# passcod/zarc

Hardware: AMD Instinct MI355X
Metric: uncompressed GiB/s (pack) at zstd -3 (higher is better)
Workload: dtype u8; 1 GPU; zarc pack 10000 x 1048576 B synthetic entries per GPU, zstd level 3, checksum on (BASELINE configs[1]); entries_per_gpu=10000, entries_total=10000, entry_bytes=1048576, level=3, kinds=text/records/lz/random round-robin

## Files before the change

zarc_amd/csrc/zge_match.hip:

```cpp
#include "zarc_device.h"
#include "zarc_kernels.h"

namespace {

#ifdef ZARC_HIPEMU
#define ZGE_CLOCK() 0ull
#else
#define ZGE_CLOCK() ((unsigned long long)__builtin_readcyclecounter())
#endif
#define ZGE_IDX(u) ((uint32_t)((wave * PER + (u)) * 64 + lane))
#ifndef ZGE_S2_DUPMASK
#define ZGE_S2_DUPMASK 0
#endif
#define ZGE_PROF(i) do { if ((dbg & 1024) && tid == 0) { const unsigned long long now_ = ZGE_CLOCK(); L.prof[i] += now_ - tprev; tprev = now_; } } while (0)

constexpr int TILE = 1024;
constexpr int THREADS = 512;
constexpr int WAVES = THREADS / 64;
constexpr int PER = TILE / THREADS;
static_assert(PER == 2, "the kernel is written for two positions per thread");
constexpr int CHUNKS = TILE / 64;
constexpr int TAG_BITS = 10;
constexpr uint32_t TAG_MASK = (1u << TAG_BITS) - 1;
struct U128 { uint64_t lo, hi; };
constexpr int CAP_MAX = 256;
constexpr int REP_BACK_MAX = 256;
constexpr int TB_BYTES = 12 + REP_BACK_MAX + TILE + CAP_MAX + 24;

template <int TAB_LOG, bool NEAR16> struct MatchLds {
    static constexpr int TAB_WORDS = NEAR16 ? (1 << TAB_LOG) / 2 : 2 << TAB_LOG;
    uint32_t tab[TAB_WORDS + (NEAR16 ? 1 : 0)];
    uint32_t a0[TILE], a1[TILE];
    uint32_t ex[TILE];
    uint32_t tb[2][(TB_BYTES + 3) / 4];
    uint32_t wcnt[CHUNKS];
    uint32_t wrep[2 * CHUNKS];
    uint32_t ctrl[16];
    unsigned long long prof[15];
};
enum { K_POS = 0, K_REP0 = 1, K_REP1 = 2, K_FLAG = 3, K_SLOT = 4, K_ANY = 5, K_CHG = 6 ,
       K_CEND = 10 ,
       K_CLEN = 11 ,
       K_LONG = 12 , K_LONG2 = 13  };

__device__ __forceinline__ uint32_t hash_long32(uint64_t v)
{
    const uint32_t lo = (uint32_t)v, hi = (uint32_t)(v >> 32);
    return lo * 0x9E3779B1u + hi * 0x85EBCA77u;
}
__device__ __forceinline__ uint32_t hash_far32(uint64_t v, uint32_t w) { return hash_long32(v) + w * 0xC2B2AE3Du; }
__device__ __forceinline__ uint32_t hash_short32(uint64_t v, int nbytes)
{
    uint32_t lo = (uint32_t)v, hi = (uint32_t)(v >> 32);
    if (nbytes < 8) hi &= (nbytes > 4) ? ((1u << (8 * (nbytes - 4))) - 1) : 0u;
    if (nbytes < 4) lo &= (1u << (8 * nbytes)) - 1;
    return lo * 0xC2B2AE3Du + hi * 0x27D4EB2Fu;
}

constexpr int REP_COST = 9;
constexpr int F_REP_BACK = 256, F_BACK_CAP = 8, F_LAZY_DELTA = 5, F_MIN_REP = 3, F_SEG_LOG = 21;
template <int MATCH_COST, int LITC> __device__ __forceinline__ int32_t score_mc(uint32_t len, uint32_t off, bool is_rep)
{
    static_assert(LITC == 5 || LITC == 6, "literal cost");
    const int32_t lits = (int32_t)((len << 2) + (LITC == 6 ? len << 1 : len));
    return is_rep ? lits - REP_COST : lits - MATCH_COST - zd::hb32(off);
}
#define score_of(P_, len_, off_, rep_) score_mc<MATCH_COST, LITC>((len_), (off_), (rep_))

template <bool WIDE> __device__ __forceinline__ uint32_t match_pack_w(uint32_t off, uint32_t len, bool rep) { return off | (len << 21) | ((rep ? 1u : 0u) << (WIDE ? 31 : 30)); }
__device__ __forceinline__ uint32_t match_off(uint32_t m) { return m & 0x1FFFFFu; }
template <bool WIDE> __device__ __forceinline__ uint32_t match_len_w(uint32_t m) { return (m >> 21) & (WIDE ? 0x3FFu : 0x1FFu); }
template <bool WIDE> __device__ __forceinline__ bool match_rep_w(uint32_t m) { return WIDE ? (m >> 31) != 0 : ((m >> 30) & 1u) != 0; }
#define match_pack(o_, l_, r_) match_pack_w<(CONT_CAP > 0 || EXT_ROUND)>((o_), (l_), (r_))
#define match_len(m_) match_len_w<(CONT_CAP > 0 || EXT_ROUND)>(m_)
#define match_rep(m_) match_rep_w<(CONT_CAP > 0 || EXT_ROUND)>(m_)
constexpr int LONG_CAP = 960;

__device__ __forceinline__ uint32_t wave_match_ext(const uint8_t *src, uint32_t p, uint32_t off, uint32_t from, uint32_t maxlen, int lane)
{
    static_assert(LONG_CAP <= 1024, "one trip of 64 x 16 bytes");
    const uint32_t at = from + 16u * (uint32_t)lane;
    const bool act = at < maxlen;
    U128 a{0, 0}, b{0, 0};
    if (act) { __builtin_memcpy(&a, src + (p + at), 16); __builtin_memcpy(&b, src + (p - off + at), 16); }
    const uint64_t xl = a.lo ^ b.lo, xh = a.hi ^ b.hi;
    const uint32_t mis = xl ? (uint32_t)(zd::ctz64(xl) >> 3) : (xh ? 8u + (uint32_t)(zd::ctz64(xh) >> 3) : 16u);
    const uint64_t bad = zd::ballot(act && mis < 16u);
    uint32_t len = maxlen;
    if (bad) {
        const uint32_t first = (uint32_t)zd::ctz64(bad);
        len = from + 16u * first + zd::readlane(mis, first);
        if (len > maxlen) len = maxlen;
    }
    return len;
}

struct StageWin { const uint32_t *w; int ndw; uint32_t wofs; };
static_assert((TB_BYTES + 3) / 4 <= THREADS, "one staged dword per thread");
__device__ __forceinline__ StageWin stage_window(const ZgeParams &P, const uint8_t *src, uint32_t n, uint32_t tile, uint32_t tend, uint32_t cap_max)
{
    (void)P;
    const uint32_t before = (uint32_t)F_REP_BACK + 8;
    const uint32_t lo = tile >= before ? tile - before : 0;
    uint32_t hi = tend + cap_max + 16;
    if (hi > n + 16) hi = n + 16;
    const uintptr_t a = (uintptr_t)(src + lo);
    const uint32_t mis = (uint32_t)(a & 3);
    StageWin s;
    s.w = (const uint32_t *)(a - mis);
    s.ndw = (int)((hi - lo + mis + 3) / 4);
    s.wofs = mis - lo;
    return s;
}

__device__ __forceinline__ uint32_t tile_end(uint32_t tile, uint32_t n)
{
    uint32_t e = tile + TILE;
    const uint32_t be = (tile / ZARC_BLOCK + 1) * ZARC_BLOCK;
    if (e > be) e = be;
    return e > n ? n : e;
}

}

template <int TAB_LOG, int SHORT_BYTES, int MATCH_COST, int F_FAR_LOG, int FAR_WAYS, bool FAR_SHORT, int FAR_STEP_LOG, int FAR_RES_LOG, int FAR_SKIP, int FAR_BACK, bool DIAG,
          bool NEAR16, int FAR_CDC, int LITC, int LAZY2, bool REP_PASS, int CONT_CAP, bool EXT_ROUND>
__device__ __forceinline__ void zge_match_body(MatchLds<TAB_LOG, NEAR16> &L, const ZgeParams &P, const uint8_t *__restrict__ src_base, const uint64_t *__restrict__ src_off,
                                               const uint64_t *__restrict__ src_len, const uint32_t *__restrict__ order, const uint32_t *__restrict__ units, uint32_t n_units,
                                               const uint64_t *__restrict__ block_prefix, ZgeBlock *__restrict__ blocks,
                                               uint64_t *__restrict__ seq_scratch, uint8_t *__restrict__ lit_scratch, uint32_t *__restrict__ queue,
                                               uint32_t *__restrict__ far_scratch)
{
    constexpr int NFAR = FAR_WAYS * (FAR_SHORT ? 2 : 1);
    constexpr int NTAB = 1 + NFAR;
    constexpr int far_shift = 32 - (F_FAR_LOG + TAG_BITS);
    constexpr uint32_t far_words = (uint32_t)(((size_t)FAR_WAYS << F_FAR_LOG) * (FAR_SHORT ? 2 : 1));
    uint32_t *const far_l = far_scratch + (size_t)blockIdx.x * far_words;
    uint32_t *const far_s = far_l + ((size_t)FAR_WAYS << F_FAR_LOG);
    constexpr uint32_t far_smask = (1u << FAR_STEP_LOG) - 1, far_rmask = (1u << FAR_RES_LOG) - 1;
    static_assert(FAR_BACK % 8 == 0 && FAR_BACK >= 8 && FAR_BACK <= 48, "backward extension of far candidates");
    static_assert(!FAR_CDC || (FAR_WAYS == 1 && !FAR_SHORT && far_shift >= FAR_CDC), "content-defined sampling: one way on the 12-byte hash");
    constexpr uint32_t cdc_mask = (1u << FAR_CDC) - 1;
    uint32_t *const Ltl = L.tab, *const Lts = L.tab + (NEAR16 ? 0 : (1 << TAB_LOG));
    typedef uint16_t __attribute__((may_alias)) u16a;
    u16a *const Lt16 = (u16a *)L.tab;
    const int tid = (int)threadIdx.x, lane = zd::lane_id();
    const uint32_t dbg = DIAG ? (uint32_t)P.dbg : 0u;
    const int wave = (int)zd::uniform((uint32_t)zd::wave_id());
    const uint64_t lt = (1ull << lane) - 1;
    const uint32_t seg_mask = (1u << F_SEG_LOG) - 1;
    const uint32_t cap_max = (uint32_t)(P.cap < CAP_MAX ? P.cap : CAP_MAX);
    unsigned long long tprev = ZGE_CLOCK();
    if (tid < 15) L.prof[tid] = 0;

    constexpr uint32_t SEG_BLOCKS = (1u << F_SEG_LOG) / ZARC_BLOCK;
    for (;;) {
    if (tid == 0) L.ctrl[K_SLOT] = atomicAdd(queue, 1u);
    zd::lds_barrier();
    const uint32_t unit = L.ctrl[K_SLOT];
    if (unit >= n_units) break;
    const uint32_t slot = units[2 * unit], ub0 = units[2 * unit + 1];
    const uint32_t f = order[slot];
    const uint8_t *src = src_base + src_off[f];
    const uint32_t n = (uint32_t)src_len[f];
    const uint32_t window = n <= (1u << P.window_log) ? (n ? n : 1u) : (1u << P.window_log);
    const uint32_t hash_end = n >= 8 ? n - 7 : 0;
    const bool far_on = NFAR && n > (uint32_t)P.far_min_frame;
    const uint32_t far_end = (far_on && n >= 12) ? n - 11 : 0;
    const uint64_t first_block = block_prefix[slot];
    const uint32_t nblocks = (uint32_t)(block_prefix[slot + 1] - first_block);

    for (int i = tid; i < MatchLds<TAB_LOG, NEAR16>::TAB_WORDS; i += THREADS) L.tab[i] = 0;
    if (NFAR && far_on) {
        uint4 *f4 = (uint4 *)far_l;
        for (uint32_t i = (uint32_t)tid; i < far_words / 4; i += THREADS) f4[i] = make_uint4(0, 0, 0, 0);
        zd::wait_vmem();
    }
    if (tid == 0) { L.ctrl[K_REP0] = 0; L.ctrl[K_REP1] = 0; }
    zd::lds_barrier();
    uint32_t cold = 0, skip_left = 0;
    constexpr bool FAR_COMPACT = FAR_RES_LOG > 0 && !FAR_CDC;
    constexpr int FNEXT_ROWS = FAR_COMPACT ? 1 : PER;
    uint32_t fnext[FNEXT_ROWS][NFAR ? NFAR : 1];
    uint32_t pf_far_tile = 0xFFFFFFFFu;
    uint32_t hfn[PER] = {0xFFFFFFFFu, 0xFFFFFFFFu};
    uint32_t pf_word = 0, pf_tile = 0xFFFFFFFFu;
    uint32_t lds_tile[2] = {0xFFFFFFFFu, 0xFFFFFFFFu};
#pragma unroll
    for (int u = 0; u < FNEXT_ROWS; u++)
#pragma unroll
        for (int k = 0; k < (NFAR ? NFAR : 1); k++) fnext[u][k] = 0;

    const uint32_t ub1 = (n > ZARC_SPLIT_MIN && ub0 + SEG_BLOCKS < nblocks) ? ub0 + SEG_BLOCKS : nblocks;
    for (uint32_t b = ub0; b < ub1; b++) {
        const uint32_t bs = b * ZARC_BLOCK;
        const uint32_t be = n - bs > ZARC_BLOCK ? bs + ZARC_BLOCK : n;
        const uint32_t blen = (uint32_t)(be - bs);
        ZgeBlock *rec = blocks + first_block + b;
        uint64_t *seq_out = seq_scratch + (first_block + b) * zge_seq_stride((uint32_t)P.slot_bytes);
        uint8_t *lit_out = lit_scratch + (first_block + b) * zge_lit_stride((uint32_t)P.slot_bytes);

        if (b > ub0 && (bs & seg_mask) == 0) {
            for (int i = tid; i < MatchLds<TAB_LOG, NEAR16>::TAB_WORDS; i += THREADS) L.tab[i] = 0;
            if (NFAR) {
                uint4 *f4 = (uint4 *)far_l;
                for (uint32_t i = (uint32_t)tid; i < far_words / 4; i += THREADS) f4[i] = make_uint4(0, 0, 0, 0);
                zd::wait_vmem();
                pf_far_tile = 0xFFFFFFFFu;
            }
        }
        if (tid == 0) { L.ctrl[K_FLAG] = 0; L.ctrl[K_POS] = 0; if (CONT_CAP) L.ctrl[K_CEND] = 0xFFFFFFFFu; }
        zd::lds_barrier();
        const uint8_t first = blen ? src[bs] : 0;
        const uint64_t pat = 0x0101010101010101ull * first;
        const uint64_t *w = (const uint64_t *)(src + bs);
        if (blen >= 1024 && tid < 128 && w[tid] != pat) L.ctrl[K_FLAG] = 1;
        zd::lds_barrier();
        if (L.ctrl[K_FLAG] == 0) {
            bool diff = false;
            const uint32_t nw = blen / 8;
            for (uint32_t i = (uint32_t)tid; i < nw; i += THREADS) diff |= w[i] != pat;
            for (uint32_t i = nw * 8 + (uint32_t)tid; i < blen; i += THREADS) diff |= src[bs + i] != first;
            if (diff) L.ctrl[K_FLAG] = 1;
        }
        zd::lds_barrier();
        const bool all_same = L.ctrl[K_FLAG] == 0;
        if (tid == 0) {
            rec->frame = f; rec->index = b; rec->src_len = blen; rec->nseq = 0; rec->nlit = 0;
            rec->type = (all_same && blen >= 2) ? 1u : 2u; rec->out_len = 0; rec->pad = 0;
        }
        if (all_same && blen >= 2) { zd::lds_barrier(); continue; }

        uint32_t nseq = 0, lp = 0;

        for (uint32_t tile = bs; tile < be; tile += TILE) {
            const uint32_t tend = be - tile > TILE ? tile + TILE : be;
            const uint32_t tcount = (uint32_t)(tend - tile);
            const uint32_t segbase = tile & ~seg_mask;
            zd::lds_barrier();
            ZGE_PROF(0);
            const uint32_t pos = bs + L.ctrl[K_POS];
            const bool cont = CONT_CAP && L.ctrl[K_CEND] == L.ctrl[K_POS] && pos >= tile;
            if (pos >= tend) { if (NFAR) zd::wait_vmem(); continue; }
            if (skip_left) {
                skip_left--;
                const uint32_t start = (uint32_t)((pos > tile ? pos : tile) - tile);
                {
                    const uint32_t cntb = tcount - start, k = (uint32_t)tid * 16;
                    const uint8_t *sp = src + tile + start;
                    uint8_t *dp = lit_out + lp;
                    if (!(dbg & 32)) {
                        if (k + 16 <= cntb) { U128 v; __builtin_memcpy(&v, sp + k, 16); __builtin_memcpy(dp + k, &v, 16); }
                        else for (uint32_t r = k; r < cntb; r++) dp[r] = sp[r];
                    }
                }
                lp += tcount - start;
                if (NFAR) zd::wait_vmem();
                zd::lds_barrier();
                if (tid == 0) L.ctrl[K_POS] = (uint32_t)(tend - bs);
                continue;
            }
            const uint32_t erep0 = L.ctrl[K_REP0], erep1 = L.ctrl[K_REP1];
            if (CONT_CAP && cont) {
                const uint32_t idx_c = pos - tile;
                if (wave == (int)(idx_c >> 7)) {
                    const uint32_t limit = (uint32_t)(be - pos);
                    uint32_t clen = 0;
                    if (erep0 != 0 && erep0 <= pos && erep0 <= window) clen = wave_match_ext(src, pos, erep0, 0, limit < (uint32_t)CONT_CAP ? limit : (uint32_t)CONT_CAP, lane);
                    if (lane == 0) L.ctrl[K_CLEN] = clen;
                }
            }
            if (tid == 0) L.ctrl[K_ANY] = 0;
            if (REP_PASS && tid < 4) L.ctrl[K_CHG + tid] = 0;
            if (EXT_ROUND && tid == 0) { L.ctrl[K_LONG] = 0; L.ctrl[K_LONG2] = 0; }

            const uint32_t bsel = (tile / TILE) & 1u;
            const uint8_t *const tbb = (const uint8_t *)L.tb[bsel];
            const uint8_t *const tbn = (const uint8_t *)L.tb[bsel ^ 1u];
            const StageWin sw = stage_window(P, src, n, tile, tend, cap_max);
            const uint32_t wofs = sw.wofs;
            const uint32_t ntile = tile + TILE;
            uint32_t wofs_n = 0;
            bool staged_now = false;
            {
                if (lds_tile[bsel] != tile) {
                    uint32_t v = pf_word;
                    if (pf_tile != tile && tid < sw.ndw) v = sw.w[tid];
                    if (tid < sw.ndw) L.tb[bsel][tid] = v;
                    lds_tile[bsel] = tile;
                    staged_now = true;
                }
                if (ntile < n) {
                    const StageWin nw = stage_window(P, src, n, ntile, tile_end(ntile, n), cap_max);
                    wofs_n = nw.wofs;
                    uint32_t v = pf_word;
                    if (pf_tile != ntile && tid < nw.ndw) v = nw.w[tid];
                    if (tid < nw.ndw) L.tb[bsel ^ 1u][tid] = v;
                    lds_tile[bsel ^ 1u] = ntile;
                    const uint32_t n2 = ntile + TILE;
                    if (n2 < n) {
                        const StageWin w2 = stage_window(P, src, n, n2, tile_end(n2, n), cap_max);
                        if (tid < w2.ndw) pf_word = w2.w[tid];
                        pf_tile = n2;
                    }
// ... 4 lines not shown
            uint64_t p8[PER];
            uint32_t fe[PER][NFAR ? NFAR : 1], ftag[PER][FAR_SHORT ? 2 : 1];
            uint32_t foffs[PER][NFAR ? NFAR : 1];
            uint64_t qf[PER][NFAR ? NFAR : 1];
            const bool far_ahead = NFAR && pf_far_tile == tile;
#pragma unroll
            for (int u = 0; u < PER; u++) {
                const uint32_t idx = ZGE_IDX(u);
                const uint32_t p = tile + idx;
                uint32_t hl = 0xFFFFFFFFu, hs = 0xFFFFFFFFu;
                p8[u] = 0;
#pragma unroll
                for (int k = 0; k < (NFAR ? NFAR : 1); k++) {
                    if (FAR_COMPACT) {
                        const uint32_t got = zd::shfl(fnext[0][k], (int)(((uint32_t)u * 64u + (uint32_t)lane) >> FAR_RES_LOG));
                        fe[u][k] = (far_ahead && !(idx & far_rmask)) ? got : 0u;
                    } else fe[u][k] = far_ahead ? fnext[FAR_COMPACT ? 0 : u][k] : 0u;
                    foffs[u][k] = 0; qf[u][k] = 0;
                }
                ftag[u][0] = 0xFFFFFFFFu;
                if (FAR_SHORT) ftag[u][1] = 0xFFFFFFFFu;
                uint32_t hfc = 0xFFFFFFFFu;
                if (idx < tcount) {
                    p8[u] = zd::load_u64(tbb + (uint32_t)(p + wofs));
                    if (p < hash_end && !(dbg & 64)) {
                        const uint32_t h32s = hash_short32(p8[u], SHORT_BYTES);
                        const uint32_t h32l = NEAR16 ? 0u : hash_long32(p8[u]);
                        hl = NEAR16 ? 0xFFFFFFFFu : h32l >> (32 - (TAB_LOG + TAG_BITS));
                        hs = NEAR16 ? h32s >> (32 - TAB_LOG) : h32s >> (32 - (TAB_LOG + TAG_BITS));
                        if (FAR_CDC) {
                            if (p < far_end && !(dbg & 2048)) {
                                if (far_ahead) hfc = hfn[u];
                                else {
                                    const uint32_t w8 = zd::load_u32(tbb + (uint32_t)(p + 8 + wofs));
                                    const uint32_t h32f = hash_far32(p8[u], w8);
                                    if (((h32f >> (far_shift - FAR_CDC)) & cdc_mask) == 0 && !((uint32_t)p8[u] == (uint32_t)(p8[u] >> 32) && (uint32_t)p8[u] == w8)) hfc = h32f >> far_shift;
                                }
                            }
                            if (hfc != 0xFFFFFFFFu) {
                                if (!far_ahead) fe[u][0] = zd::load_l2_u32(far_l + (size_t)(hfc >> TAG_BITS));
                                else {
                                    const uint32_t e = fe[u][0];
                                    uint32_t o = (e && (e & TAG_MASK) == (hfc & TAG_MASK) && !(dbg & 4096)) ? p - (segbase + (e >> TAG_BITS) - 1) : 0u;
                                    if (o + 8 > p || o > window || (dbg & 1)) o = 0;
                                    foffs[u][0] = o;
                                    if (o) qf[u][0] = zd::load_u64(src + (p - o));
                                }
                            }
                        } else
                        if (NFAR && p < far_end && !(p & far_rmask) && !(dbg & 2048)) {
                            const uint32_t hf = (h32l + zd::load_u32(tbb + (uint32_t)(p + 8 + wofs)) * 0xC2B2AE3Du) >> far_shift, hg = h32s >> far_shift;
                            ftag[u][0] = hf & TAG_MASK;
                            if (FAR_SHORT) ftag[u][1] = hg & TAG_MASK;
                            if (!far_ahead) {
                                if (FAR_WAYS == 2) {
                                    const uint64_t el = zd::load_l2_u64(far_l + (size_t)(hf >> TAG_BITS) * 2);
                                    fe[u][0] = (uint32_t)el; fe[u][1] = (uint32_t)(el >> 32);
                                    if (FAR_SHORT) { const uint64_t es = zd::load_l2_u64(far_s + (size_t)(hg >> TAG_BITS) * 2); fe[u][2] = (uint32_t)es; fe[u][3] = (uint32_t)(es >> 32); }
                                } else {
#pragma unroll
                                for (int w = 0; w < FAR_WAYS; w++) {
                                    fe[u][w] = zd::load_l2_u32(far_l + ((size_t)(hf >> TAG_BITS) * FAR_WAYS + w));
                                    if (FAR_SHORT) fe[u][FAR_WAYS + w] = zd::load_l2_u32(far_s + ((size_t)(hg >> TAG_BITS) * FAR_WAYS + w));
                                }
                                }
                            } else {
#pragma unroll
                                for (int k = 0; k < NFAR; k++) {
                                    const uint32_t e = fe[u][k];
                                    uint32_t o = (e && (e & TAG_MASK) == ftag[u][k / (FAR_WAYS ? FAR_WAYS : 1)] && !(dbg & 4096)) ? p - (segbase + (e >> TAG_BITS) - 1) : 0u;
#pragma unroll
                                    for (int j = 0; j < k; j++) if (o == foffs[u][j]) o = 0;
                                    if (o + 8 > p || o > window || (dbg & 1)) o = 0;
                                    foffs[u][k] = o;
                                    if (o) qf[u][k] = zd::load_u64(src + (p - o));
                                }
                            }
                        }
                    }
                }
                L.a0[idx] = NEAR16 ? (hs == 0xFFFFFFFFu ? (1u << TAB_LOG) : hs) : hl;
                if (!NEAR16) L.a1[idx] = hs;
                else if (FAR_CDC) L.a1[idx] = hfc;
                L.ex[idx] = 0;
            }
            zd::lds_barrier();
            ZGE_PROF(2);
            if (NEAR16) {
              if (wave == 0 && !(dbg & 4)) {
                zd::wave_priority<3>();
                uint32_t h[CHUNKS], e[CHUNKS];
#if ZGE_S2_DUPMASK
                uint64_t dupmask = 0;
#endif
#pragma unroll
                for (int k = 0; k < CHUNKS; k++) {
                    h[k] = L.a0[k * 64 + lane];
#if ZGE_S2_DUPMASK
                    const uint32_t hn = lane < 63 ? L.a0[k * 64 + lane + 1] : 0xFFFFFFFFu;
                    if (hn == h[k]) dupmask |= 1ull << k;
#endif
                }
#pragma unroll
                for (int k = 0; k < CHUNKS; k++) {
                    e[k] = (uint32_t)Lt16[h[k]];
                    zd::wave_lds_order();
#if ZGE_S2_DUPMASK
                    if (!((dupmask >> k) & 1))
#endif
                    Lt16[h[k]] = (uint16_t)((uint32_t)tile + (uint32_t)(k * 64 + lane));
                    zd::wave_lds_order();
                }
#pragma unroll
                for (int k = 0; k < CHUNKS; k++) L.a0[k * 64 + lane] = e[k];
                zd::wave_priority<0>();
              }
            } else
            if (wave < 2 && !(dbg & 4)) {
                zd::wave_priority<3>();
                uint32_t *tab = wave == 0 ? Ltl : Lts;
                uint32_t *hc = wave == 0 ? L.a0 : L.a1;
                uint32_t h[CHUNKS], e[CHUNKS];
                uint64_t dupmask = 0;
#pragma unroll
                for (int k = 0; k < CHUNKS; k++) {
                    h[k] = hc[k * 64 + lane];
                    const uint32_t hn = lane < 63 ? hc[k * 64 + lane + 1] : 0xFFFFFFFFu;
                    if (hn == h[k]) dupmask |= 1ull << k;
                }
#pragma unroll
                for (int k = 0; k < CHUNKS; k++) {
                    const bool act = h[k] != 0xFFFFFFFFu;
                    e[k] = act ? tab[h[k] >> TAG_BITS] : 0u;
                    zd::wave_lds_order();
                    if (act && !((dupmask >> k) & 1)) {
                        const uint32_t code = ((uint32_t)(tile - segbase) + (uint32_t)(k * 64 + lane) + 1) << TAG_BITS;
                        atomicMax(&tab[h[k] >> TAG_BITS], code | (h[k] & TAG_MASK));
                    }
                    zd::wave_lds_order();
                }
#pragma unroll
                for (int k = 0; k < CHUNKS; k++)
                    hc[k * 64 + lane] = e[k] ^ (h[k] & TAG_MASK);
                zd::wave_priority<0>();
            }
            if (NFAR) zd::wait_vmem();
            zd::lds_barrier();
            ZGE_PROF(3);
            uint32_t near_e[PER] = {0, 0};
            if (FAR_CDC) {
                uint64_t vnx[PER];
                uint32_t wnx[PER];
#pragma unroll
                for (int u = 0; u < PER; u++) {
                    const uint32_t pn = ntile + ZGE_IDX(u);
                    const uint32_t at = pn < far_end ? (uint32_t)(pn + wofs_n) : 0u;
                    vnx[u] = zd::load_u64(tbn + at);
                    wnx[u] = zd::load_u32(tbn + at + 8);
                    if (NEAR16) near_e[u] = L.a0[ZGE_IDX(u)];
                }
#pragma unroll
                for (int u = 0; u < PER; u++) {
                    const uint32_t pn = ntile + ZGE_IDX(u);
                    hfn[u] = 0xFFFFFFFFu;
                    fnext[u][0] = 0;
                    if (pn < far_end && !(dbg & (2048 | 32768))) {
                        const uint64_t vn = vnx[u];
// ... 202 lines not shown
                        else { if (sc > b_score[0]) { b_score[0] = sc; b_len[0] = clen; b_off[0] = erep0; b_flags[0] = 1u | 4u; } }
                    }
                }
            }
#pragma unroll
            for (int u = 0; u < PER; u++) {
                const uint32_t idx = ZGE_IDX(u);
                const uint32_t p = tile + idx;
                const uint32_t best_len = b_len[u], best_off = b_off[u];
                const int32_t best_score = b_score[u];
                const bool best_rep = b_flags[u] & 1u, from_guess = b_flags[u] & 2u, best_fol = b_flags[u] & 4u, best_far = b_flags[u] & 8u;
                if (best_len && best_score > 0) {
                    const uint32_t q = p - best_off;
                    const uint32_t bcap = (NFAR && best_far) ? (uint32_t)FAR_BACK : (uint32_t)F_BACK_CAP;
                    uint32_t maxb = bcap;
                    if (p - bs < maxb) maxb = (uint32_t)(p - bs);
                    uint32_t back = 0;
                    if (maxb && q >= bcap && !best_fol) {
                        uint64_t best_before = q16[u].lo;
                        if (from_guess) best_before = zd::load_u64(tbb + (uint32_t)(q - 8 + wofs));
                        if (NFAR && best_far) best_before = zd::load_u64(src + (q - 8));
                        const uint64_t x = zd::load_u64(tbb + (uint32_t)(p - 8 + wofs)) ^ best_before;
                        back = x ? (uint32_t)(__clzll((long long)x) >> 3) : 8u;
                        if (NFAR && FAR_BACK > 8 && best_far) {
#pragma unroll
                            for (uint32_t j = 16; j <= (uint32_t)FAR_BACK; j += 8) {
                                if (back == j - 8 && maxb > j - 8) {
                                    const uint64_t x2 = zd::load_u64(tbb + (uint32_t)(p - j + wofs)) ^ zd::load_u64(src + (q - j));
                                    back += x2 ? (uint32_t)(__clzll((long long)x2) >> 3) : 8u;
                                }
                            }
                        }
                        if (back > maxb) back = maxb;
                    }
                    mo[u] = best_off;
                    mw[u] = best_len | (back << 16) | ((best_rep ? 1u : 0u) << 24);
                }
            }
            ZGE_PROF(11);
#pragma unroll
            for (int u = 0; u < PER; u++) L.a0[ZGE_IDX(u)] = match_pack(mo[u], mw[u] & 0xFFFF, (mw[u] >> 24) & 1);
            if (mo[0] | mo[1]) L.ctrl[K_ANY] = 1;
            if (EXT_ROUND) {
                const uint32_t r0 = (mw[0] & 0xFFFFu) + ((mw[0] >> 16) & 0xFFu), r1 = (mw[1] & 0xFFFFu) + ((mw[1] >> 16) & 0xFFu);
                if ((r0 > r1 ? r0 : r1) >= cap_max) L.ctrl[K_LONG] = 1;
            }
            uint32_t fo[PER], fw[PER];
            uint64_t msel[PER], mlit[PER];
            {
#define ZGE_FIRST 1
#include "zge_parse_round.h"
#undef ZGE_FIRST
            }
            if (EXT_ROUND && L.ctrl[K_LONG]) {
                uint64_t extm[PER];
                bool any = false;
#pragma unroll
                for (int u = 0; u < PER; u++) {
                    const uint32_t idx = ZGE_IDX(u);
                    const uint32_t flen = fw[u] & 0xFFFFu, lim = idx < tcount ? (uint32_t)(be - tile) - idx : 0u;
                    extm[u] = msel[u] & zd::ballot(flen >= cap_max && lim > flen);
                    any |= extm[u] != 0;
                }
                if (any && lane == 0) L.ctrl[K_LONG2] = 1;
                zd::lds_barrier();
                if (L.ctrl[K_LONG2]) {
#pragma unroll
                for (int u = 0; u < PER; u++) {
                    const uint32_t idx = ZGE_IDX(u);
                    const uint32_t p = tile + idx;
                    const uint32_t flen = fw[u] & 0xFFFFu;
                    uint64_t ext = extm[u];
                    while (ext) {
                        const uint32_t who = (uint32_t)zd::ctz64(ext);
                        ext &= ext - 1;
                        const uint32_t p_w = zd::readlane(p, who), len_w = zd::readlane(flen, who), off_w = zd::readlane(fo[u], who);
                        const uint32_t lim_w = (uint32_t)(be - p_w), maxl = lim_w < (uint32_t)LONG_CAP ? lim_w : (uint32_t)LONG_CAP;
                        if (maxl > len_w) {
                            const uint32_t e = wave_match_ext(src, p_w, off_w, len_w, maxl, lane);
                            if ((uint32_t)lane == who && e > len_w) { mo[u] = fo[u]; mw[u] = e | (fw[u] & (1u << 24)); }
                        }
                    }
                    L.a0[idx] = match_pack(mo[u], mw[u] & 0xFFFF, (mw[u] >> 24) & 1);
                    L.ex[idx] = 0;
                }
                zd::lds_barrier();
                {
#define ZGE_FIRST 0
#include "zge_parse_round.h"
#undef ZGE_FIRST
                }
                }
            }
            if (REP_PASS) for (uint32_t it = 0; it < (uint32_t)P.rep_pass; it++) {
            {
                const uint32_t wr = L.wrep[lane & 31];
                uint32_t sl = erep0, sl1 = erep1;
                for (int c = 0; c < wave * PER; c++) {
                    const uint32_t cl = zd::readlane(wr, (uint32_t)(2 * c)), cd = zd::readlane(wr, (uint32_t)(2 * c + 1));
                    if (cl) { if (cd) { sl1 = cd; sl = cl; } else if (cl != sl) { sl1 = sl; sl = cl; } }
                }
                uint32_t lv[PER], lv1[PER];
#pragma unroll
                for (int u = 0; u < PER; u++) {
                    lv[u] = sl; lv1[u] = sl1;
                    uint64_t rem = msel[u];
                    while (rem) {
                        const uint32_t q = (uint32_t)zd::ctz64(rem);
                        rem &= rem - 1;
                        const uint32_t o = zd::readlane(fo[u], q);
                        if (o != sl) { sl1 = sl; sl = o; }
                        if ((uint32_t)lane > q) { lv[u] = sl; lv1[u] = sl1; }
                    }
                }
                uint64_t onpath[PER];
#pragma unroll
                for (int u = 0; u < PER; u++) { const uint64_t mk = msel[u] | mlit[u]; onpath[u] = mk | (mk << 1); }
                U128 qa[PER][2];
                bool ok[PER][2];
                bool changed = false;
#pragma unroll
                for (int u = 0; u < PER; u++) {
                    const uint32_t idx = ZGE_IDX(u);
                    const uint32_t p = tile + idx;
#pragma unroll
                    for (int k = 0; k < 2; k++) {
                        const uint32_t lo = k ? lv1[u] : lv[u];
                        ok[u][k] = idx < tcount && lo != 0 && lo + 8 <= p && lo <= window && !(k && lv1[u] == lv[u]) && ((onpath[u] >> lane) & 1);
                        qa[u][k] = U128{0, 0};
                        if (ok[u][k]) __builtin_memcpy(&qa[u][k], src + (p - lo - 8), 16);
                    }
                }
#pragma unroll
                for (int u = 0; u < PER; u++) {
                    const uint32_t idx = ZGE_IDX(u);
                    const uint32_t p = tile + idx;
                    const uint32_t limit = idx < tcount ? (uint32_t)(be - p) : 0u, cap = limit < cap_max ? limit : cap_max;
                    uint32_t olen = mw[u] & 0xFFFF;
                    int32_t cur = olen ? score_of(P, olen, mo[u], (mw[u] >> 24) & 1) : 0;
#pragma unroll
                    for (int k = 0; k < 2; k++) {
                        if (!ok[u][k]) continue;
                        const uint32_t lo = k ? lv1[u] : lv[u];
                        const uint32_t len = prefix_len(p, p8[u], cap, lo, qa[u][k].hi);
                        if (len < (uint32_t)F_MIN_REP) continue;
                        const int32_t sc = score_of(P, len, lo, true);
                        if (sc > cur) {
                            cur = sc;
                            uint32_t maxb = (uint32_t)F_BACK_CAP;
                            if (p - bs < maxb) maxb = (uint32_t)(p - bs);
                            const uint64_t x = zd::load_u64(tbb + (uint32_t)(p - 8 + wofs)) ^ qa[u][k].lo;
                            uint32_t back = x ? (uint32_t)(__clzll((long long)x) >> 3) : 8u;
                            if (back > maxb) back = maxb;
                            mo[u] = lo;
                            mw[u] = len | (back << 16) | (1u << 24);
                            changed = true;
                        }
                    }
                    if (CONT_CAP) {
                        const uint32_t flen = fw[u] & 0xFFFFu;
                        uint64_t ext = msel[u] & zd::ballot(flen >= cap_max);
                        while (ext) {
                            const uint32_t who = (uint32_t)zd::ctz64(ext);
                            ext &= ext - 1;
                            const uint32_t p_w = zd::readlane(p, who), len_w = zd::readlane(flen, who), off_w = zd::readlane(fo[u], who);
                            const uint32_t lim_w = (uint32_t)(be - p_w), maxl = lim_w < (uint32_t)CONT_CAP ? lim_w : (uint32_t)CONT_CAP;
                            if (maxl > len_w) {
                                const uint32_t e = wave_match_ext(src, p_w, off_w, len_w, maxl, lane);
                                if ((uint32_t)lane == who && e > len_w) { mo[u] = fo[u]; mw[u] = e | (fw[u] & (1u << 24)); changed = true; }
                            }
                        }
                    }
                    L.a0[idx] = match_pack(mo[u], mw[u] & 0xFFFF, (mw[u] >> 24) & 1);
                    L.ex[idx] = 0;
                }
                if (changed) L.ctrl[K_CHG + it] = 1;
            }
            zd::lds_barrier();
            ZGE_PROF(14);
            if (L.ctrl[K_CHG + it] == 0) break;
            {
#define ZGE_FIRST 0
#include "zge_parse_round.h"
#undef ZGE_FIRST
            }
            }
            uint32_t sel_total, lit_total, sel_before[PER], lit_before[PER];
            {
                static_assert(CHUNKS == 16, "the chunk counts are scanned inside one 16-lane row");
                const uint32_t cv = zd::row_scan_incl(lane < CHUNKS ? L.wcnt[lane] : 0u);
                const uint32_t tot = zd::readlane(cv, CHUNKS - 1);
                sel_total = tot >> 16;
                lit_total = tot & 0xFFFFu;
#pragma unroll
                for (int u = 0; u < PER; u++) {
                    const uint32_t incl = zd::readlane(cv, (uint32_t)(wave * PER + u));
                    sel_before[u] = (incl >> 16) - (uint32_t)__popcll(msel[u]);
                    lit_before[u] = (incl & 0xFFFFu) - (uint32_t)__popcll(mlit[u]);
                }
            }
#pragma unroll
            for (int u = 0; u < PER; u++) {
                const uint32_t my_sel_idx = sel_before[u] + (uint32_t)__popcll(msel[u] & lt);
                const uint32_t my_lit_idx = lit_before[u] + (uint32_t)__popcll(mlit[u] & lt);
                if (dbg & 32) continue;
                if ((msel[u] >> lane) & 1) {
                    seq_out[nseq + my_sel_idx] = zge_pack_seq(lp + my_lit_idx, fw[u] & 0xFFFF, fo[u]);
                    if (my_sel_idx + 1 == sel_total) { L.ctrl[K_REP0] = fo[u]; if (sel_total == 1) L.ctrl[K_REP1] = erep0; if (CONT_CAP) L.ctrl[K_CEND] = (uint32_t)(tile - bs) + ZGE_IDX(u) + (fw[u] & 0xFFFF); }
                    if (my_sel_idx + 2 == sel_total) L.ctrl[K_REP1] = fo[u];
                }
                if ((mlit[u] >> lane) & 1) lit_out[lp + my_lit_idx] = (uint8_t)p8[u];
            }
            nseq += sel_total;
            lp += lit_total;
            ZGE_PROF(8);
        }
        if (tid == 0) { rec->nseq = nseq; rec->nlit = lp; }
        if (NFAR) zd::wait_vmem();
        zd::lds_barrier();
    }
    }
    if ((dbg & 1024) && tid < 15) atomicAdd((unsigned long long *)(queue + 2) + tid, L.prof[tid]);
}
#undef score_of
#undef match_pack
#undef match_len
#undef match_rep

__global__ void __launch_bounds__(512, 4) zarc_zge_match(ZgeParams P, const uint8_t *__restrict__ src_base, const uint64_t *__restrict__ src_off,
                                                      const uint64_t *__restrict__ src_len, const uint32_t *__restrict__ order, const uint32_t *__restrict__ units, uint32_t n_units,
                                                      const uint64_t *__restrict__ block_prefix, ZgeBlock *__restrict__ blocks,
                                                      uint64_t *__restrict__ seq_scratch, uint8_t *__restrict__ lit_scratch, uint32_t *__restrict__ queue,
                                                      uint32_t *__restrict__ far_scratch)
{
    __shared__ MatchLds<15, true> L;
    zge_match_body<15, 5, 12, 16, 1, false, 5, 2, 64, 48, false, true, 4, 5, 0, false, 0, true>(L, P, src_base, src_off, src_len, order, units, n_units, block_prefix, blocks, seq_scratch, lit_scratch, queue, far_scratch);
}

__global__ void __launch_bounds__(512, 4) zarc_zge_match_fast(ZgeParams P, const uint8_t *__restrict__ src_base, const uint64_t *__restrict__ src_off,
                                                           const uint64_t *__restrict__ src_len, const uint32_t *__restrict__ order, const uint32_t *__restrict__ units, uint32_t n_units,
                                                           const uint64_t *__restrict__ block_prefix, ZgeBlock *__restrict__ blocks,
                                                           uint64_t *__restrict__ seq_scratch, uint8_t *__restrict__ lit_scratch, uint32_t *__restrict__ queue,
                                                           uint32_t *__restrict__ far_scratch)
{
    __shared__ MatchLds<15, true> L;
    zge_match_body<15, 5, 12, 0, 0, false, 0, 0, 0, 8, false, true, 0, 5, 0, false, 0, false>(L, P, src_base, src_off, src_len, order, units, n_units, block_prefix, blocks, seq_scratch, lit_scratch, queue, far_scratch);
}

#ifdef ZARC_GPU_DIAG
__global__ void __launch_bounds__(512, 4) zarc_zge_match_diag(ZgeParams P, const uint8_t *__restrict__ src_base, const uint64_t *__restrict__ src_off,
                                                           const uint64_t *__restrict__ src_len, const uint32_t *__restrict__ order, const uint32_t *__restrict__ units, uint32_t n_units,
                                                           const uint64_t *__restrict__ block_prefix, ZgeBlock *__restrict__ blocks,
                                                           uint64_t *__restrict__ seq_scratch, uint8_t *__restrict__ lit_scratch, uint32_t *__restrict__ queue,
                                                           uint32_t *__restrict__ far_scratch)
{
    __shared__ MatchLds<15, true> L;
    zge_match_body<15, 5, 12, 16, 1, false, 5, 2, 64, 48, true, true, 4, 5, 0, false, 0, true>(L, P, src_base, src_off, src_len, order, units, n_units, block_prefix, blocks, seq_scratch, lit_scratch, queue, far_scratch);
}
#endif

__global__ void __launch_bounds__(512, 2) zarc_zge_match_deep(ZgeParams P, const uint8_t *__restrict__ src_base, const uint64_t *__restrict__ src_off,
                                                           const uint64_t *__restrict__ src_len, const uint32_t *__restrict__ order, const uint32_t *__restrict__ units, uint32_t n_units,
                                                           const uint64_t *__restrict__ block_prefix, ZgeBlock *__restrict__ blocks,
                                                           uint64_t *__restrict__ seq_scratch, uint8_t *__restrict__ lit_scratch, uint32_t *__restrict__ queue,
                                                           uint32_t *__restrict__ far_scratch)
{
    __shared__ MatchLds<13, false> L;
    zge_match_body<13, 4, 10, 16, 2, true, 1, 0, 0, 48, false, false, 0, 6, 5, true, LONG_CAP, false>(L, P, src_base, src_off, src_len, order, units, n_units, block_prefix, blocks, seq_scratch, lit_scratch, queue, far_scratch);
}

#ifdef ZARC_GPU_DIAG
__global__ void __launch_bounds__(512, 2) zarc_zge_match_deep_diag(ZgeParams P, const uint8_t *__restrict__ src_base, const uint64_t *__restrict__ src_off,
                                                           const uint64_t *__restrict__ src_len, const uint32_t *__restrict__ order, const uint32_t *__restrict__ units, uint32_t n_units,
                                                           const uint64_t *__restrict__ block_prefix, ZgeBlock *__restrict__ blocks,
                                                           uint64_t *__restrict__ seq_scratch, uint8_t *__restrict__ lit_scratch, uint32_t *__restrict__ queue,
                                                           uint32_t *__restrict__ far_scratch)
{
    __shared__ MatchLds<13, false> L;
    zge_match_body<13, 4, 10, 16, 2, true, 1, 0, 0, 48, true, false, 0, 6, 5, true, LONG_CAP, false>(L, P, src_base, src_off, src_len, order, units, n_units, block_prefix, blocks, seq_scratch, lit_scratch, queue, far_scratch);
}
#endif
```

zarc_amd/csrc/zge_parse_round.h:

```cpp
#pragma unroll
            for (int u = 0; u < PER; u++) {
                const uint32_t idx = ZGE_IDX(u);
                const uint32_t len = mw[u] & 0xFFFF, back = (mw[u] >> 16) & 0xFF;
                if (len && back && !(dbg & 8)) {
                    const bool rep = (mw[u] >> 24) & 1;
                    const int32_t base = score_of(P, len, mo[u], rep);
                    const uint32_t lim = back < idx ? back : idx;
#pragma unroll
                    for (uint32_t k = 1; k <= (uint32_t)F_BACK_CAP; k++) {
                        const int32_t sc = base + LITC * (int32_t)k;
                        if (k <= lim && sc > 0) atomicMax(&L.ex[idx - k], ((uint32_t)sc << 6) | (63u - k));
                    }
                    for (uint32_t k = (uint32_t)F_BACK_CAP + 1; k <= lim; k++) {
                        const int32_t sc = base + LITC * (int32_t)k;
                        if (sc > 0) atomicMax(&L.ex[idx - k], ((uint32_t)sc << 6) | (63u - k));
                    }
                }
            }
#if ZGE_FIRST
                ZGE_PROF(12);
                if (NFAR) zd::wait_vmem();
                ZGE_PROF(13);
#endif
            zd::lds_barrier();
#if ZGE_FIRST
            ZGE_PROF(4);
            if (NFAR) {
                const uint32_t way = (tile / TILE) & (uint32_t)(FAR_WAYS - 1);
#pragma unroll
                for (int u = 0; u < PER; u++) {
                    const uint32_t idx = ZGE_IDX(u);
                    const uint32_t p = tile + idx;
                    if (FAR_CDC) {
                        const uint32_t hfc = L.a1[idx];
                        if (hfc != 0xFFFFFFFFu && !(dbg & (64 | 8192)))
                            zd::atomic_max_l2(far_l + (size_t)(hfc >> TAG_BITS), ((((uint32_t)(tile - segbase) + idx + 1) << TAG_BITS)) | (hfc & TAG_MASK));
                    } else
                    if (idx < tcount && p < far_end && (p & far_smask) <= far_rmask && !(dbg & (64 | 8192))) {
                        const uint32_t code = ((uint32_t)(tile - segbase) + idx + 1) << TAG_BITS;
                        const uint32_t hf = hash_far32(p8[u], zd::load_u32(tbb + (uint32_t)(p + 8 + wofs))) >> far_shift;
                        zd::atomic_max_l2(far_l + ((size_t)(hf >> TAG_BITS) * FAR_WAYS + way), code | (hf & TAG_MASK));
                        if (FAR_SHORT) {
                            const uint32_t hg = hash_short32(p8[u], SHORT_BYTES) >> far_shift;
                            zd::atomic_max_l2(far_s + ((size_t)(hg >> TAG_BITS) * FAR_WAYS + way), code | (hg & TAG_MASK));
                        }
                    }
                }
            }
            if (L.ctrl[K_ANY] == 0) {
                const uint32_t start = (uint32_t)((pos > tile ? pos : tile) - tile);
#pragma unroll
                for (int u = 0; u < PER; u++) {
                    const uint32_t idx = ZGE_IDX(u);
                    if (idx >= start && idx < tcount && !(dbg & 32)) lit_out[lp + (idx - start)] = (uint8_t)p8[u];
                }
                lp += tcount - start;
                if (tid == 0) { L.ctrl[K_POS] = (uint32_t)(tend - bs); if (CONT_CAP) L.ctrl[K_CEND] = 0xFFFFFFFFu; }
                cold++;
                if (cold >= 2) skip_left = cold >= 4 ? 7u : (1u << (cold - 1)) - 1;
                if (NFAR) zd::wait_vmem();
                continue;
            }
            cold = 0;
#endif
#pragma unroll
            for (int u = 0; u < PER; u++) {
                const uint32_t idx = ZGE_IDX(u);
                const uint32_t offer = L.ex[idx];
                uint32_t blen_ = mw[u] & 0xFFFF, boff = mo[u];
                bool brep = (mw[u] >> 24) & 1;
                if (offer) {
                    const int32_t own = blen_ ? score_of(P, blen_, boff, brep) : 0;
                    if ((int32_t)(offer >> 6) > own) {
                        const uint32_t k = 63u - (offer & 63u);
                        const uint32_t nm = L.a0[idx + k];
                        boff = match_off(nm);
                        blen_ = match_len(nm) + k;
                        brep = match_rep(nm);
                    }
                }
                fo[u] = boff;
                fw[u] = blen_ | ((brep ? 1u : 0u) << 24);
                L.a1[idx] = match_pack(boff, blen_, brep);
            }
            zd::lds_barrier();
            ZGE_PROF(5);
            bool take[PER];
            uint32_t nx[PER];
#pragma unroll
            for (int u = 0; u < PER; u++) {
                const uint32_t idx = ZGE_IDX(u);
                const uint32_t my_len = fw[u] & 0xFFFF;
                take[u] = idx < tcount && my_len != 0;
                if (take[u] && P.lazy && idx + 1 < tcount) {
                    const uint32_t m2 = L.a1[idx + 1];
                    const uint32_t l2 = match_len(m2);
                    if (l2 && score_of(P, l2, match_off(m2), match_rep(m2)) > score_of(P, my_len, fo[u], (fw[u] >> 24) & 1) + F_LAZY_DELTA) take[u] = false;
                }
                if (LAZY2 && take[u] && idx + 2 < tcount) {
                    const uint32_t m3 = L.a1[idx + 2];
                    const uint32_t l3 = match_len(m3);
                    if (l3 && score_of(P, l3, match_off(m3), match_rep(m3)) > score_of(P, my_len, fo[u], (fw[u] >> 24) & 1) + LAZY2) take[u] = false;
                }
                nx[u] = take[u] ? idx + my_len : idx + 1;
            }
            {
                uint32_t val[PER];
#pragma unroll
                for (int u = 0; u < PER; u++) {
                    const uint32_t cbase = (uint32_t)(wave * PER + u) * 64;
                    const uint32_t cend = cbase + 64 < tcount ? cbase + 64 : tcount;
                    val[u] = nx[u];
#pragma unroll
                    for (int r = 0; r < 6; r++) {
                        const uint32_t v2 = zd::shfl(val[u], (int)((val[u] - cbase) & 63));
                        if (val[u] < cend) val[u] = v2;
                    }
                }
                {
                    const uint32_t obase = (uint32_t)(wave * PER + 1) * 64, oend = obase + 64 < tcount ? obase + 64 : tcount;
                    const uint32_t through = zd::shfl(val[1], (int)((val[0] - obase) & 63));
                    if (val[0] >= obase && val[0] < oend) val[0] = through;
                }
#pragma unroll
                for (int u = 0; u < PER; u++) L.ex[ZGE_IDX(u)] = val[u];
            }
            zd::lds_barrier();
            ZGE_PROF(6);
            {
                zd::wave_priority<2>();
                uint32_t cur = (uint32_t)((pos > tile ? pos : tile) - tile);
                int c = 0;
#pragma unroll
                for (; c < wave; c++) {
                    const uint32_t pend = (uint32_t)(c * 128 + 128) < tcount ? (uint32_t)(c * 128 + 128) : tcount;
                    if (cur < pend) cur = L.ex[cur];
                }
                cur = zd::uniform(cur);
#pragma unroll
                for (int u = 0; u < PER; u++) {
                    const int mychunk = wave * PER + u;
                    const uint32_t cbase = (uint32_t)mychunk * 64;
                    const uint32_t cend = cbase + 64 < tcount ? cbase + 64 : tcount;
                    const uint64_t tk = zd::ballot(take[u]);
                    const uint32_t span = cend > cbase ? cend - cbase : 0u;
                    uint64_t sel = 0, lits = 0;
                    const uint32_t entry = cur;
                    uint32_t o_last = 0, o_diff = 0;
                    if (!(dbg & 2)) {
                        while (cur < cend) {
                            const uint64_t ahead = tk & (~0ull << (cur - cbase));
                            if (ahead == 0) { cur = cend; break; }
                            const uint32_t q = (uint32_t)zd::ctz64(ahead);
                            sel |= 1ull << q;
                            cur = zd::readlane(nx[u], q);
                            if (REP_PASS) { const uint32_t o = zd::readlane(fo[u], q); if (o != o_last) { o_diff = o_last; o_last = o; } }
                        }
                        const uint64_t below = sel & lt;
                        const uint32_t qs = below ? 63u - (uint32_t)__clzll((long long)below) : 0u;
                        const uint32_t over = zd::shfl(nx[u], (int)qs);
                        const uint32_t me = cbase + (uint32_t)lane;
                        lits = zd::ballot(me >= entry && (uint32_t)lane < span && !((sel >> lane) & 1) && (!below || over <= me));
                    }
                    msel[u] = sel;
                    mlit[u] = lits;
                    if (lane == 0) L.wcnt[mychunk] = ((uint32_t)__popcll(msel[u]) << 16) | (uint32_t)__popcll(mlit[u]);
// ... 8 lines not shown
```

Baseline: 42.78 GiB/s.

## Replace scatter atomicMax backward offers with gather over neighbor words

Each position now writes one packed word (score, position-adjusted, and lookback limit) into the ex array. Readers gather the next eight words plus, for far backward extents, ballot-driven wave broadcasts, and take the best offer. This replaces up to eight LDS atomicMax scatters per match and removes the per-round zeroing of ex. The LDS struct is reordered, wrep is shrunk when REP_PASS is off, and the uniform-block check reads through load_u64. The cost is more LDS reads per position and a more intricate encoding, which could change parse results if the score arithmetic differs.

```diff
diff --git a/zarc_amd/csrc/zge_match.hip b/zarc_amd/csrc/zge_match.hip
--- a/zarc_amd/csrc/zge_match.hip
+++ b/zarc_amd/csrc/zge_match.hip
@@ -27,15 +27,15 @@
 constexpr int REP_BACK_MAX = 256;
 constexpr int TB_BYTES = 12 + REP_BACK_MAX + TILE + CAP_MAX + 24;
 
-template <int TAB_LOG, bool NEAR16> struct MatchLds {
+template <int TAB_LOG, bool NEAR16, bool REP_PASS> struct MatchLds {
     static constexpr int TAB_WORDS = NEAR16 ? (1 << TAB_LOG) / 2 : 2 << TAB_LOG;
+    uint32_t a0[TILE], a1[TILE];
+    uint32_t ex[TILE + 8];
+    uint32_t wcnt[CHUNKS];
+    uint32_t wrep[REP_PASS ? 2 * CHUNKS : 1];
+    uint32_t ctrl[16];
+    uint32_t tb[2][(TB_BYTES + 3) / 4];
     uint32_t tab[TAB_WORDS + (NEAR16 ? 1 : 0)];
-    uint32_t a0[TILE], a1[TILE];
-    uint32_t ex[TILE];
-    uint32_t tb[2][(TB_BYTES + 3) / 4];
-    uint32_t wcnt[CHUNKS];
-    uint32_t wrep[2 * CHUNKS];
-    uint32_t ctrl[16];
     unsigned long long prof[15];
 };
 enum { K_POS = 0, K_REP0 = 1, K_REP1 = 2, K_FLAG = 3, K_SLOT = 4, K_ANY = 5, K_CHG = 6 ,
@@ -75,6 +75,46 @@
 #define match_len(m_) match_len_w<(CONT_CAP > 0 || EXT_ROUND)>(m_)
 #define match_rep(m_) match_rep_w<(CONT_CAP > 0 || EXT_ROUND)>(m_)
 constexpr int LONG_CAP = 960;
+
+template <bool FAR, class LDS> __device__ __forceinline__ void bwd_gather(const LDS &L, uint32_t (&bw)[PER], int wave, int lane)
+{
+    static_assert(F_BACK_CAP == 8 && sizeof(L.ex) == (TILE + F_BACK_CAP) * 4, "eight words after every position");
+    uint32_t own[PER];
+#pragma unroll
+    for (int u = 0; u < PER; u++) {
+        const uint32_t idx = (uint32_t)((wave * PER + u) * 64 + lane);
+        uint32_t w[F_BACK_CAP + 1];
+#pragma unroll
+        for (int k = 0; k <= F_BACK_CAP; k++) w[k] = L.ex[idx + (uint32_t)k];
+        uint32_t b = 0;
+#pragma unroll
+        for (int k = 1; k <= F_BACK_CAP; k++) {
+            const uint32_t c = (w[k] & 63u) >= (uint32_t)k ? w[k] : 0u;
+            b = c > b ? c : b;
+        }
+        bw[u] = b;
+        own[u] = w[0];
+    }
+    if (FAR) {
+        const uint32_t nxt = wave < WAVES - 1 ? L.ex[(uint32_t)((wave * PER + PER) * 64 + lane)] : 0u;
+        const uint64_t m0 = zd::ballot((own[0] & 63u) > (uint32_t)F_BACK_CAP), m1 = zd::ballot((own[1] & 63u) > (uint32_t)F_BACK_CAP);
+        const uint64_t m2 = zd::ballot((nxt & 63u) > (uint32_t)F_BACK_CAP);
+        if (m0 | m1 | m2) {
+            const uint32_t c0 = (uint32_t)(wave * PER) * 64u;
+            auto take = [&](int u, uint32_t s, uint32_t ws) {
+                const uint32_t k = s - (c0 + (uint32_t)u * 64u + (uint32_t)lane);
+                if (k - 9u <= (ws & 63u) - 9u && ws > bw[u]) bw[u] = ws;
+            };
+            for (uint64_t m = m0; m; m &= m - 1) { const uint32_t q = (uint32_t)zd::ctz64(m); take(0, c0 + q, zd::readlane(own[0], q)); }
+            for (uint64_t m = m1; m; m &= m - 1) {
+                const uint32_t q = (uint32_t)zd::ctz64(m), ws = zd::readlane(own[1], q);
+                take(0, c0 + 64u + q, ws);
+                take(1, c0 + 64u + q, ws);
+            }
+            for (uint64_t m = m2; m; m &= m - 1) { const uint32_t q = (uint32_t)zd::ctz64(m); take(1, c0 + 128u + q, zd::readlane(nxt, q)); }
+        }
+    }
+}
 
 __device__ __forceinline__ uint32_t wave_match_ext(const uint8_t *src, uint32_t p, uint32_t off, uint32_t from, uint32_t maxlen, int lane)
 {
@@ -125,7 +165,7 @@
 
 template <int TAB_LOG, int SHORT_BYTES, int MATCH_COST, int F_FAR_LOG, int FAR_WAYS, bool FAR_SHORT, int FAR_STEP_LOG, int FAR_RES_LOG, int FAR_SKIP, int FAR_BACK, bool DIAG,
           bool NEAR16, int FAR_CDC, int LITC, int LAZY2, bool REP_PASS, int CONT_CAP, bool EXT_ROUND>
-__device__ __forceinline__ void zge_match_body(MatchLds<TAB_LOG, NEAR16> &L, const ZgeParams &P, const uint8_t *__restrict__ src_base, const uint64_t *__restrict__ src_off,
+__device__ __forceinline__ void zge_match_body(MatchLds<TAB_LOG, NEAR16, REP_PASS> &L, const ZgeParams &P, const uint8_t *__restrict__ src_base, const uint64_t *__restrict__ src_off,
                                                const uint64_t *__restrict__ src_len, const uint32_t *__restrict__ order, const uint32_t *__restrict__ units, uint32_t n_units,
                                                const uint64_t *__restrict__ block_prefix, ZgeBlock *__restrict__ blocks,
                                                uint64_t *__restrict__ seq_scratch, uint8_t *__restrict__ lit_scratch, uint32_t *__restrict__ queue,
@@ -141,6 +181,7 @@
     static_assert(FAR_BACK % 8 == 0 && FAR_BACK >= 8 && FAR_BACK <= 48, "backward extension of far candidates");
     static_assert(!FAR_CDC || (FAR_WAYS == 1 && !FAR_SHORT && far_shift >= FAR_CDC), "content-defined sampling: one way on the 12-byte hash");
     constexpr uint32_t cdc_mask = (1u << FAR_CDC) - 1;
+    constexpr uint32_t BWD_D = 64u * (uint32_t)LITC - 1u;
     uint32_t *const Ltl = L.tab, *const Lts = L.tab + (NEAR16 ? 0 : (1 << TAB_LOG));
     typedef uint16_t __attribute__((may_alias)) u16a;
     u16a *const Lt16 = (u16a *)L.tab;
@@ -152,6 +193,7 @@
     const uint32_t cap_max = (uint32_t)(P.cap < CAP_MAX ? P.cap : CAP_MAX);
     unsigned long long tprev = ZGE_CLOCK();
     if (tid < 15) L.prof[tid] = 0;
+    if (tid < F_BACK_CAP) L.ex[TILE + tid] = 0;
 
     constexpr uint32_t SEG_BLOCKS = (1u << F_SEG_LOG) / ZARC_BLOCK;
     for (;;) {
@@ -170,7 +212,7 @@
     const uint64_t first_block = block_prefix[slot];
     const uint32_t nblocks = (uint32_t)(block_prefix[slot + 1] - first_block);
 
-    for (int i = tid; i < MatchLds<TAB_LOG, NEAR16>::TAB_WORDS; i += THREADS) L.tab[i] = 0;
+    for (int i = tid; i < MatchLds<TAB_LOG, NEAR16, REP_PASS>::TAB_WORDS; i += THREADS) L.tab[i] = 0;
     if (NFAR && far_on) {
         uint4 *f4 = (uint4 *)far_l;
         for (uint32_t i = (uint32_t)tid; i < far_words / 4; i += THREADS) f4[i] = make_uint4(0, 0, 0, 0);
@@ -201,7 +243,7 @@
         uint8_t *lit_out = lit_scratch + (first_block + b) * zge_lit_stride((uint32_t)P.slot_bytes);
 
         if (b > ub0 && (bs & seg_mask) == 0) {
-            for (int i = tid; i < MatchLds<TAB_LOG, NEAR16>::TAB_WORDS; i += THREADS) L.tab[i] = 0;
+            for (int i = tid; i < MatchLds<TAB_LOG, NEAR16, REP_PASS>::TAB_WORDS; i += THREADS) L.tab[i] = 0;
             if (NFAR) {
                 uint4 *f4 = (uint4 *)far_l;
                 for (uint32_t i = (uint32_t)tid; i < far_words / 4; i += THREADS) f4[i] = make_uint4(0, 0, 0, 0);
@@ -219,7 +261,7 @@
         if (L.ctrl[K_FLAG] == 0) {
             bool diff = false;
             const uint32_t nw = blen / 8;
-            for (uint32_t i = (uint32_t)tid; i < nw; i += THREADS) diff |= w[i] != pat;
+            for (uint32_t i = (uint32_t)tid; i < nw; i += THREADS) diff |= zd::load_u64(src + (bs + 8u * i)) != pat;
             for (uint32_t i = nw * 8 + (uint32_t)tid; i < blen; i += THREADS) diff |= src[bs + i] != first;
             if (diff) L.ctrl[K_FLAG] = 1;
         }
@@ -390,7 +432,6 @@
                 L.a0[idx] = NEAR16 ? (hs == 0xFFFFFFFFu ? (1u << TAB_LOG) : hs) : hl;
                 if (!NEAR16) L.a1[idx] = hs;
                 else if (FAR_CDC) L.a1[idx] = hfc;
-                L.ex[idx] = 0;
             }
             zd::lds_barrier();
             ZGE_PROF(2);
@@ -759,7 +800,6 @@
                         }
                     }
                     L.a0[idx] = match_pack(mo[u], mw[u] & 0xFFFF, (mw[u] >> 24) & 1);
-                    L.ex[idx] = 0;
                 }
                 zd::lds_barrier();
                 {
@@ -849,7 +889,6 @@
                         }
                     }
                     L.a0[idx] = match_pack(mo[u], mw[u] & 0xFFFF, (mw[u] >> 24) & 1);
-                    L.ex[idx] = 0;
                 }
                 if (changed) L.ctrl[K_CHG + it] = 1;
             }
@@ -910,7 +949,7 @@
                                                       uint64_t *__restrict__ seq_scratch, uint8_t *__restrict__ lit_scratch, uint32_t *__restrict__ queue,
                                                       uint32_t *__restrict__ far_scratch)
 {
-    __shared__ MatchLds<15, true> L;
+    __shared__ MatchLds<15, true, false> L;
     zge_match_body<15, 5, 12, 16, 1, false, 5, 2, 64, 48, false, true, 4, 5, 0, false, 0, true>(L, P, src_base, src_off, src_len, order, units, n_units, block_prefix, blocks, seq_scratch, lit_scratch, queue, far_scratch);
 }
 
@@ -920,7 +959,7 @@
                                                            uint64_t *__restrict__ seq_scratch, uint8_t *__restrict__ lit_scratch, uint32_t *__restrict__ queue,
                                                            uint32_t *__restrict__ far_scratch)
 {
-    __shared__ MatchLds<15, true> L;
+    __shared__ MatchLds<15, true, false> L;
     zge_match_body<15, 5, 12, 0, 0, false, 0, 0, 0, 8, false, true, 0, 5, 0, false, 0, false>(L, P, src_base, src_off, src_len, order, units, n_units, block_prefix, blocks, seq_scratch, lit_scratch, queue, far_scratch);
 }
 
@@ -931,7 +970,7 @@
                                                            uint64_t *__restrict__ seq_scratch, uint8_t *__restrict__ lit_scratch, uint32_t *__restrict__ queue,
                                                            uint32_t *__restrict__ far_scratch)
 {
-    __shared__ MatchLds<15, true> L;
+    __shared__ MatchLds<15, true, false> L;
     zge_match_body<15, 5, 12, 16, 1, false, 5, 2, 64, 48, true, true, 4, 5, 0, false, 0, true>(L, P, src_base, src_off, src_len, order, units, n_units, block_prefix, blocks, seq_scratch, lit_scratch, queue, far_scratch);
 }
 #endif
@@ -942,7 +981,7 @@
                                                            uint64_t *__restrict__ seq_scratch, uint8_t *__restrict__ lit_scratch, uint32_t *__restrict__ queue,
                                                            uint32_t *__restrict__ far_scratch)
 {
-    __shared__ MatchLds<13, false> L;
+    __shared__ MatchLds<13, false, true> L;
     zge_match_body<13, 4, 10, 16, 2, true, 1, 0, 0, 48, false, false, 0, 6, 5, true, LONG_CAP, false>(L, P, src_base, src_off, src_len, order, units, n_units, block_prefix, blocks, seq_scratch, lit_scratch, queue, far_scratch);
 }
 
@@ -953,7 +992,7 @@
                                                            uint64_t *__restrict__ seq_scratch, uint8_t *__restrict__ lit_scratch, uint32_t *__restrict__ queue,
                                                            uint32_t *__restrict__ far_scratch)
 {
-    __shared__ MatchLds<13, false> L;
+    __shared__ MatchLds<13, false, true> L;
     zge_match_body<13, 4, 10, 16, 2, true, 1, 0, 0, 48, true, false, 0, 6, 5, true, LONG_CAP, false>(L, P, src_base, src_off, src_len, order, units, n_units, block_prefix, blocks, seq_scratch, lit_scratch, queue, far_scratch);
 }
 #endif
diff --git a/zarc_amd/csrc/zge_parse_round.h b/zarc_amd/csrc/zge_parse_round.h
--- a/zarc_amd/csrc/zge_parse_round.h
+++ b/zarc_amd/csrc/zge_parse_round.h
@@ -2,20 +2,13 @@
             for (int u = 0; u < PER; u++) {
                 const uint32_t idx = ZGE_IDX(u);
                 const uint32_t len = mw[u] & 0xFFFF, back = (mw[u] >> 16) & 0xFF;
+                uint32_t word = 0;
                 if (len && back && !(dbg & 8)) {
-                    const bool rep = (mw[u] >> 24) & 1;
-                    const int32_t base = score_of(P, len, mo[u], rep);
+                    const int32_t base = score_of(P, len, mo[u], (mw[u] >> 24) & 1);
                     const uint32_t lim = back < idx ? back : idx;
-#pragma unroll
-                    for (uint32_t k = 1; k <= (uint32_t)F_BACK_CAP; k++) {
-                        const int32_t sc = base + LITC * (int32_t)k;
-                        if (k <= lim && sc > 0) atomicMax(&L.ex[idx - k], ((uint32_t)sc << 6) | (63u - k));
-                    }
-                    for (uint32_t k = (uint32_t)F_BACK_CAP + 1; k <= lim; k++) {
-                        const int32_t sc = base + LITC * (int32_t)k;
-                        if (sc > 0) atomicMax(&L.ex[idx - k], ((uint32_t)sc << 6) | (63u - k));
-                    }
+                    word = (((uint32_t)base * 64u + 63u + idx * BWD_D) << 6) | lim;
                 }
+                L.ex[idx] = word;
             }
 #if ZGE_FIRST
                 ZGE_PROF(12);
@@ -63,10 +56,13 @@
             }
             cold = 0;
 #endif
+            {
+            uint32_t bw[PER];
+            bwd_gather<(FAR_BACK > F_BACK_CAP)>(L, bw, wave, lane);
 #pragma unroll
             for (int u = 0; u < PER; u++) {
                 const uint32_t idx = ZGE_IDX(u);
-                const uint32_t offer = L.ex[idx];
+                const uint32_t offer = bw[u] ? (bw[u] >> 6) - idx * BWD_D : 0u;
                 uint32_t blen_ = mw[u] & 0xFFFF, boff = mo[u];
                 bool brep = (mw[u] >> 24) & 1;
                 if (offer) {
@@ -82,6 +78,7 @@
                 fo[u] = boff;
                 fw[u] = blen_ | ((brep ? 1u : 0u) << 24);
                 L.a1[idx] = match_pack(boff, blen_, brep);
+            }
             }
             zd::lds_barrier();
             ZGE_PROF(5);
```

After: 42.82 GiB/s, median of 6. About the same (+0.1%).
